# arpitbansal297/Cold-Diffusion-Models

Measured on AMD Instinct MI355X. Metric: unet_train_imgs_per_sec, higher is better.
Workload: dtype f32 storage/accumulate; dense-conv GEMM operands bf16x3; 1 GPU; CelebA-128 denoising cold diffusion (BASELINE config 3): Unet(dim=64,(1,2,4,8),ch=3) @128x128, T=200, optimizer step = 2 micro-batches x 32 img (one fused forward / backward pass over all of them: same draws, same gradient sum) + Adam + EMA/10; per_gpu_batch=32, gradient_accumulate_every=2, parallelism=single

## Files before the change

### cold-diffusion-models_amd/csrc/cdf_common.h

```cpp
#pragma once
#include <stdint.h>
#include <stddef.h>

#ifdef CDF_EMU
#include "hipemu.h"
#else
#include <hip/hip_runtime.h>
#define CDF_LAUNCH(kernel, grid, block, shmem, stream, ...) \
    hipLaunchKernelGGL(kernel, grid, block, shmem, stream, __VA_ARGS__)
#define CDF_DYN_SMEM(name) extern __shared__ __attribute__((aligned(16))) unsigned char name[]
#define CDF_LDS_BARRIER() asm volatile("s_waitcnt lgkmcnt(0)\n\ts_barrier" ::: "memory")
#define CDF_GLDS16(gptr, lds_base)                                                                            \
    __builtin_amdgcn_global_load_lds((const __attribute__((address_space(1))) void*)(gptr),                    \
                                     (__attribute__((address_space(3))) void*)(lds_base), 16, 0, 0)
#define CDF_WAIT_DMA() asm volatile("s_waitcnt vmcnt(0)" ::: "memory")
#define CDF_WAIT_DMA_LEAVE(N) asm volatile("s_waitcnt vmcnt(%0)" ::"n"(N) : "memory")
#define CDF_SCHED_FENCE() __builtin_amdgcn_sched_barrier(0)
#define CDF_WAIT_LDS() __builtin_amdgcn_s_waitcnt(0xC07F)
typedef float f32x4_t __attribute__((ext_vector_type(4)));
typedef float f32x16_t __attribute__((ext_vector_type(16)));
#endif
#ifdef CDF_EMU
#define CDF_LAUNCH_LDS_MAX(max_bytes, kernel, grid, block, shmem, stream, ...) CDF_LAUNCH(kernel, grid, block, shmem, stream, __VA_ARGS__)
#else
// ... 191 lines not shown
#define CDF_IO_RES_BF16 1
#define CDF_IO_PRE_BF16 2
#define CDF_IO_MUL_BF16 4
#define CDF_IO_PRE_GRAD 8

#define CDF_OK 0
#define CDF_E_INVALID (-1)
#define CDF_E_UNSUPPORTED (-2)
#define CDF_E_LAUNCH (-3)

#define CDF_WAVE 64
#define CDF_S ((hipStream_t)stream)

void cdf_set_error(const char* fmt, ...);
int cdf_check_launch(const char* what);

#define CDF_REQUIRE(cond, ...)                  \
    do {                                        \
        if (!(cond)) {                          \
            cdf_set_error(__VA_ARGS__);         \
            return CDF_E_INVALID;               \
        }                                       \
    } while (0)

static inline int cdf_cdiv(long long a, long long b) { return (int)((a + b - 1) / b); }

__device__ __forceinline__ int cdf_xcd_order(int bid, int nblk) {
    const int q = nblk >> 3, r = nblk & 7;
    const int xcd = bid & 7, idx = bid >> 3;
    const int base = xcd < r ? xcd * (q + 1) : r * (q + 1) + (xcd - r) * q;
// ... 65 lines not shown
```

### cold-diffusion-models_amd/csrc/k_conv.hip

```cpp
#include <atomic>
#include "cdf_common.h"
#include "cdf_epilogue.h"
#include "colddiff.h"

#define CDF_MAX_TAPS 16

struct ConvPhase {
    int oy, ox, ntaps;
    signed char dy[CDF_MAX_TAPS], dx[CDF_MAX_TAPS], wi[CDF_MAX_TAPS];
};

struct ConvArgs {
    const float* x;
    const float* w;
    float* y;
    const float* bias;
    const float* sbias;
    const float* res;
    float* pre;
    const float* mul;
    int ldx, ldw, ldy, ld_sbias, ldr, ldp, ldm;
    int B, H, W, Cin, OH, OW, Cout, QH, QW, os, is;
    int act;
    int mul_mode;
// ... 365 lines not shown
                           : a.out + (((long long)split * a.nbatch + batch) * a.ntaps + tap) * a.CA * a.ldo;
#pragma unroll
    for (int i = 0; i < MT; ++i)
#pragma unroll
        for (int r = 0; r < 16; ++r) {
            const int ca = tile_a * BMC + wm * WM + i * 32 + cdf_acc_row(r, half);
            if (ca >= a.CA) continue;
#pragma unroll
            for (int j = 0; j < NT; ++j) {
                const int cb = tile_b * BNC + wn * WN + j * 32 + l31;
                if (cb < a.ldo) O[(long long)ca * a.ldo + cb] = cb < a.CB ? acc[i][j][r] : 0.f;
            }
        }
}

__global__ void pack_weight_kernel(const float* src, float* dst, int T, int R, int C, int ldc, long long s_t,
                                   long long s_r, long long s_c) {
    const long long n = (long long)T * R * ldc;
    for (long long i = (long long)blockIdx.x * blockDim.x + threadIdx.x; i < n; i += (long long)gridDim.x * blockDim.x) {
        const int c = (int)(i % ldc);
        const long long tr = i / ldc;
        const int r = (int)(tr % R), t = (int)(tr / R);
        dst[i] = c < C ? src[c * s_c + r * s_r + t * s_t] : 0.f;
    }
}
template <int SL>
__global__ void __launch_bounds__(64 * SL) unpack_reduce_kernel(const float* ws, float* g, int nsplit, int T, int R, int C, int ldc,
                                                                long long s_t, long long s_r, long long s_c, int accumulate,
                                                                const float* bws, float* gb, int bC, int bld) {
    __shared__ float red[SL][64];
    if (bws != nullptr && blockIdx.y == 1) {
        ws = bws; g = gb; T = 1; R = 1; C = bC; ldc = bld; s_t = 0; s_r = 0; s_c = 1;
    }
    const long long n = (long long)T * R * C;
    const long long slab = (long long)T * R * ldc;
    const int l = threadIdx.x & 63, rl = threadIdx.x >> 6;
    for (long long base = (long long)blockIdx.x * 64; base < n; base += (long long)gridDim.x * 64) {
        const long long i = base + l;
        float s0 = 0.f, s1 = 0.f, s2 = 0.f, s3 = 0.f;
        int c = 0, r = 0, t = 0;
// ... 43 lines not shown
        tr = tile / tiles_c;
        tc = tile - tr * tiles_c;
    }
    const int c0 = tc * 32, r0 = tr * RJ;
    const long long slab = (long long)T_ * R * ldc;
    const int cc = c0 + cl < C ? c0 + cl : C - 1;
    int roff[J];
#pragma unroll
    for (int j = 0; j < J; ++j) {
        const int r = r0 + j / T_, t = j % T_;
        roff[j] = (t * R + (r < R ? r : R - 1)) * ldc + cc;
    }
    float acc[J];
#pragma unroll
    for (int j = 0; j < J; ++j) acc[j] = 0.f;
    for (int z = zg; z < nsplit; z += 8) {
        const float* p = ws + (long long)z * slab;
        float v[J];
#pragma unroll
        for (int j = 0; j < J; ++j) v[j] = p[roff[j]];
#pragma unroll
        for (int j = 0; j < J; ++j) acc[j] += v[j];
    }
#pragma unroll
    for (int j = 0; j < J; ++j) red[(zg * J + j) * 33 + cl] = acc[j];
    __syncthreads();
    constexpr int NE = (32 * J + 255) / 256;
    float tot[NE], old[NE];
    float* dst[NE];
    bool ok[NE];
#pragma unroll
// ... 55 lines not shown
        for (; r < r1; r += 4) s += cdf_widen(p[(long long)r * ld + c]);
    }
    red[rl][threadIdx.x & 63] = s;
    __syncthreads();
    if (rl == 0 && c < C) {
        const int l = threadIdx.x;
        part[((long long)blockIdx.y * gridDim.z + blockIdx.z) * C + c] = (red[0][l] + red[1][l]) + (red[2][l] + red[3][l]);
    }
}
__global__ void __launch_bounds__(1024) colsum_final_kernel(const float* part, float* out, int nchunk, int C, int ldo, int accumulate) {
    __shared__ float red[16][64];
    const int l = threadIdx.x & 63, rl = threadIdx.x >> 6, c = blockIdx.x * 64 + l;
    float s = 0.f;
    if (c < C) {
        const float* p = part + (long long)blockIdx.y * nchunk * C + c;
        for (int k = rl; k < nchunk; k += 16) s += p[(long long)k * C];
    }
    red[rl][l] = s;
    __syncthreads();
    if (rl == 0 && c < C) {
        float t = 0.f;
#pragma unroll
        for (int r = 0; r < 16; ++r) t += red[r][l];
        float* dst = out + (long long)blockIdx.y * ldo + c;
        *dst = accumulate ? *dst + t : t;
    }
}

static int check_feat(const char* who, const void* p, int ld, int C) {
    CDF_REQUIRE(p != nullptr, "%s: null tensor", who);
    CDF_REQUIRE((((uintptr_t)p) & 15) == 0, "%s: tensor not 16-byte aligned", who);
// ... 142 lines not shown

static inline int ew_grid2(long long n) {
    long long g = (n + 255) / 256;
    if (g > 4096) g = 4096;
    return g < 1 ? 1 : (int)g;
}

struct CdfPackEntry {
    const float* src;
    void* dst0;
    void* dst1;
    long long s_t, s_r, s_c;
    int T, R, C, ldc, kind, first_block;
};

__global__ void __launch_bounds__(256) pack_many_kernel(const CdfPackEntry* tab, int nentries) {
    int lo = 0, hi = nentries - 1;
    const int b = blockIdx.x;
    while (lo < hi) {
        const int mid = (lo + hi + 1) >> 1;
        if (tab[mid].first_block <= b) lo = mid; else hi = mid - 1;
    }
    const CdfPackEntry e = tab[lo];
    if (e.s_t == 1 && e.T > 1 && e.T <= 16) {
        const long long n2 = (long long)e.R * e.ldc;
        const long long j0 = (long long)(b - e.first_block) * 1024 + threadIdx.x;
        const long long plane = (long long)e.R * e.ldc;
#pragma unroll
        for (int k = 0; k < 4; ++k) {
            const long long j = j0 + 256 * k;
            if (j >= n2) break;
            const int c = (int)(j % e.ldc), r = (int)(j / e.ldc);
            const bool ok = c < e.C;
            const float* sp = e.src + (ok ? c * e.s_c + r * e.s_r : 0);
            float v[16];
#pragma unroll
            for (int t = 0; t < 16; ++t) v[t] = sp[t < e.T ? t : 0];
#pragma unroll
            for (int t = 0; t < 16; ++t) {
                if (t >= e.T) break;
                const float x = ok ? v[t] : 0.f;
                const long long i = t * plane + j;
                if (e.kind == 0) {
                    ((float*)e.dst0)[i] = x;
                } else {
                    const unsigned h = cdf_f2bf(x);
                    ((unsigned short*)e.dst0)[i] = (unsigned short)h;
                    if (e.dst1) ((unsigned short*)e.dst1)[i] = (unsigned short)cdf_f2bf(x - cdf_bf2f(h));
                }
            }
        }
        return;
    }
    const long long n = (long long)e.T * e.R * e.ldc;
    const long long i0 = (long long)(b - e.first_block) * 1024 + threadIdx.x;
#pragma unroll
    for (int k = 0; k < 4; ++k) {
        const long long i = i0 + 256 * k;
        if (i >= n) break;
        const int c = (int)(i % e.ldc);
        const long long tr = i / e.ldc;
        const int r = (int)(tr % e.R), t = (int)(tr / e.R);
        const float v = c < e.C ? e.src[c * e.s_c + r * e.s_r + t * e.s_t] : 0.f;
        if (e.kind == 0) {
            ((float*)e.dst0)[i] = v;
        } else {
            const unsigned h = cdf_f2bf(v);
            ((unsigned short*)e.dst0)[i] = (unsigned short)h;
            if (e.dst1) ((unsigned short*)e.dst1)[i] = (unsigned short)cdf_f2bf(v - cdf_bf2f(h));
        }
    }
}

extern "C" int cdf_pack_entry_bytes(void) { return (int)sizeof(CdfPackEntry); }
extern "C" int cdf_pack_blocks(int T, int R, int ldc, long long s_t) {
    const long long n = (s_t == 1 && T > 1 && T <= 16) ? (long long)R * ldc : (long long)T * R * ldc;
    return (int)((n + 1023) / 1024);
}

extern "C" int cdf_pack_many(const void* table, int nentries, int nblocks, void* stream) {
    CDF_REQUIRE(table && nentries > 0 && nblocks > 0, "cdf_pack_many: bad args");
    CDF_LAUNCH(pack_many_kernel, dim3(nblocks), dim3(256), 0, CDF_S, (const CdfPackEntry*)table, nentries);
    return cdf_check_launch("pack_many");
}

extern "C" int cdf_pack_weight(const float* src, float* dst, int T, int R, int C, int ldc, long long s_t,
                               long long s_r, long long s_c, void* stream) {
    CDF_REQUIRE(src && dst && T > 0 && R > 0 && C > 0 && ldc >= C && ldc % 4 == 0, "cdf_pack_weight: bad args");
    CDF_LAUNCH(pack_weight_kernel, dim3(ew_grid2((long long)T * R * ldc)), dim3(256), 0, CDF_S, src, dst, T, R, C, ldc, s_t, s_r, s_c);
    return cdf_check_launch("pack_weight");
}

static int launch_unpack_reduce(const float* ws, float* g, int nsplit, int T, int R, int C, int ldc, long long s_t, long long s_r,
                                long long s_c, int accumulate, const float* bws, float* gb, int bC, int bld, int tiled, hipStream_t s) {
    const int tiled_mode = tiled ? 1 : 0;
    if (s_c != 1 && C >= 32 && (T == 1 || T == 9 || T == 16) && tiled_mode) {
        const int RJ = T == 9 ? 4 : (T == 16 ? 2 : 32);
        const long long tiles = (long long)((C + 31) / 32) * ((R + RJ - 1) / RJ);
        if (tiles < (1 << 30) && (!bws || (bC + 31) / 32 <= tiles)) {
            const dim3 tg((unsigned)tiles, bws ? 2 : 1);
            if (T == 9)
                CDF_LAUNCH((unpack_reduce_tiled_kernel<9, 4>), tg, dim3(256), 0, s, ws, g, nsplit, R, C, ldc, s_t, s_r, s_c, accumulate, bws, gb, bC, bld, tiled_mode);
            else if (T == 16)
                CDF_LAUNCH((unpack_reduce_tiled_kernel<16, 2>), tg, dim3(256), 0, s, ws, g, nsplit, R, C, ldc, s_t, s_r, s_c, accumulate, bws, gb, bC, bld, tiled_mode);
            else
                CDF_LAUNCH((unpack_reduce_tiled_kernel<1, 32>), tg, dim3(256), 0, s, ws, g, nsplit, R, C, ldc, s_t, s_r, s_c, accumulate, bws, gb, bC, bld, tiled_mode);
            return cdf_check_launch("unpack_reduce_tiled");
        }
    }
    const dim3 grid(ew_grid2((long long)T * R * C * 4), bws ? 2 : 1);
    if (nsplit >= 32)
        CDF_LAUNCH(unpack_reduce_kernel<16>, grid, dim3(1024), 0, s, ws, g, nsplit, T, R, C, ldc, s_t, s_r, s_c, accumulate, bws, gb, bC, bld);
    else
        CDF_LAUNCH(unpack_reduce_kernel<4>, grid, dim3(256), 0, s, ws, g, nsplit, T, R, C, ldc, s_t, s_r, s_c, accumulate, bws, gb, bC, bld);
    return cdf_check_launch("unpack_reduce");
}

extern "C" int cdf_unpack_reduce(const float* ws, float* g, int nsplit, int T, int R, int C, int ldc, long long s_t,
                                 long long s_r, long long s_c, int accumulate, int tiled, void* stream) {
// ... 35 lines not shown
```

### cold-diffusion-models_amd/csrc/k_conv_sp.hip

```cpp
#include "cdf_conv_sp.h"
#include <atomic>

template <int SPLIT>
__global__ void __launch_bounds__(256, 2) conv_igemm_sp_kernel(SpArgs a) {
    constexpr int BM = 128, BN = 128, BK = 32, AS = 40;
    constexpr int NPL = SPLIT == 1 ? 1 : 2;
    constexpr int PLANE = BM * AS;
    constexpr int STAGE = 2 * NPL * PLANE;
    CDF_DYN_SMEM(smem_raw);
    unsigned short* smem = (unsigned short*)smem_raw;

    const int tid = threadIdx.x, lane = tid & 63, wave = tid >> 6;
    const int wm = wave >> 1, wn = wave & 1;
    const int M = a.B * a.QH * a.QW;
    const int tiles_n = (a.Cout + BN - 1) / BN, tiles_m = (M + BM - 1) / BM;
    const int tile = cdf_sp_swizzle(blockIdx.x, tiles_m * tiles_n);
    const int tile_m = tile / tiles_n, tile_n = tile - tile_m * tiles_n;
    const SpPhase& ph = a.ph[blockIdx.y];

    const int a_c4 = (tid & 7) * 4;
    int a_iy0[4], a_ix0[4];
    unsigned a_pix[4];
#pragma unroll
    for (int p = 0; p < 4; ++p) {
// ... 473 lines not shown
            }
        }
        __syncthreads();
    }
    psum += __shfl_xor(psum, 32);
    float* fold = stg;
    if (ctx_wave) {
        cdf_acc_stage(fold, LD, ch * LD, 0, cacc, half, l31);
        if (half == 0) fold[4 * LD * LD + ch * LD + l31] = psum;
    }
    __syncthreads();
    const size_t pb = (size_t)b * a.P + p;
    for (int e = tid; e < 4 * LD * LD; e += 512) a.ctx_part[pb * 4 * (LD * LD) + e] = t_lo < t_hi ? fold[e] : 0.f;
    if (tid < HD) a.sum_part[pb * HD + tid] = t_lo < t_hi ? fold[4 * LD * LD + tid] : 0.f;
    if (ctx_wave && half == 0) a.max_part[pb * HD + ch * LD + l31] = m_run;
}

__global__ void pack_weight_bf16_kernel(const float* src, unsigned short* dst_hi, unsigned short* dst_lo, int T, int R, int C,
                                        int ldc, long long s_t, long long s_r, long long s_c) {
    const long long n = (long long)T * R * ldc;
    for (long long i = (long long)blockIdx.x * blockDim.x + threadIdx.x; i < n; i += (long long)gridDim.x * blockDim.x) {
        const int c = (int)(i % ldc);
        const long long tr = i / ldc;
        const int r = (int)(tr % R), t = (int)(tr / R);
        const float v = c < C ? src[c * s_c + r * s_r + t * s_t] : 0.f;
        const unsigned h = cdf_f2bf(v);
        dst_hi[i] = (unsigned short)h;
        if (dst_lo) dst_lo[i] = (unsigned short)cdf_f2bf(v - cdf_bf2f(h));
    }
}

extern "C" int cdf_linattn_kvctx_parts(int B, int n, int slots) {
    const int tiles = n / 128;
    if (tiles < 1 || B < 1) return 0;
    int P = (slots > 0 ? slots : 512) / B;
    if (P < 1) P = 1;
    if (P > tiles) P = tiles;
    const int tpb = (tiles + P - 1) / P;
    return (tiles + tpb - 1) / tpb;
}

extern "C" int cdf_linattn_kvctx(const float* xn, int ldx, const void* w_hi, const void* w_lo, int ldk, float* kv, int ldkv, float* ws, int B,
                                 int n, int dim, int heads, int slots, void* stream) {
    CDF_REQUIRE(xn && w_hi && kv && ws && B > 0, "cdf_linattn_kvctx: null pointer");
// ... 12 lines not shown
    a.tiles_per_block = (tiles + P - 1) / P;
    const size_t lds = (size_t)128 * (256 + 8) * sizeof(float) + 8 * 32 * sizeof(float);
    if (dim % 64 == 0) {
        if (w_lo) CDF_LAUNCH_LDS((linattn_kvctx_kernel<3, 64>), dim3(P, B), dim3(512), lds, CDF_S, a);
        else CDF_LAUNCH_LDS((linattn_kvctx_kernel<1, 64>), dim3(P, B), dim3(512), lds, CDF_S, a);
    } else {
        if (w_lo) CDF_LAUNCH_LDS((linattn_kvctx_kernel<3, 32>), dim3(P, B), dim3(512), lds, CDF_S, a);
        else CDF_LAUNCH_LDS((linattn_kvctx_kernel<1, 32>), dim3(P, B), dim3(512), lds, CDF_S, a);
    }
    return cdf_check_launch("linattn_kvctx");
}

extern "C" int cdf_pack_weight_bf16(const float* src, void* dst_hi, void* dst_lo, int T, int R, int C, int ldc, long long s_t,
                                    long long s_r, long long s_c, void* stream) {
    CDF_REQUIRE(src && dst_hi && T > 0 && R > 0 && C > 0 && ldc >= C && ldc % 32 == 0, "cdf_pack_weight_bf16: bad args (ldc must be a multiple of 32)");
    long long g = ((long long)T * R * ldc + 255) / 256;
    if (g > 4096) g = 4096;
    CDF_LAUNCH(pack_weight_bf16_kernel, dim3((int)g), dim3(256), 0, CDF_S, src, (unsigned short*)dst_hi, (unsigned short*)dst_lo, T, R, C, ldc, s_t, s_r, s_c);
    return cdf_check_launch("pack_weight_bf16");
}

extern "C" int cdf_conv_gemm_bf16(const float* x, int ldx, const void* w_hi, const void* w_lo, int ldk, float* y, int ldy, int B,
                                  int H, int W, int Cin, int OH, int OW, int Cout, int QH, int QW, int os, int is, int nphase,
                                  const int* phase_desc, const float* bias, const float* sbias, int ld_sbias, const float* res,
                                  int ldr, float* pre, int ldp, const float* mul, int ldm, int act, int mul_mode, int accumulate,
                                  int split, void* stream) {
    CDF_REQUIRE(x && w_hi && y && (((uintptr_t)x) & 15) == 0 && ldx % 4 == 0 && ldx >= Cin, "cdf_conv_gemm_bf16: bad x");
    CDF_REQUIRE((split == 1 || split == 3) && (split == 1 || w_lo), "cdf_conv_gemm_bf16: split must be 1 (bf16) or 3 (hi/lo bf16x3)");
    CDF_REQUIRE((((uintptr_t)w_hi) & 15) == 0 && ldk % 32 == 0 && ldk >= Cin, "cdf_conv_gemm_bf16: weights must be 16B aligned with ldk %% 32 == 0");
    CDF_REQUIRE(nphase >= 1 && nphase <= 4 && phase_desc && ldy >= Cout, "cdf_conv_gemm_bf16: bad geometry");
    CDF_REQUIRE(!mul_mode || mul, "cdf_conv_gemm_bf16: mul_mode without mul tensor");
    SpArgs a;
    a.x = x; a.w_hi = (const unsigned short*)w_hi; a.w_lo = (const unsigned short*)w_lo; a.y = y;
    a.bias = bias; a.sbias = sbias; a.res = res; a.pre = pre; a.mul = mul;
// ... 72 lines not shown
```

### cold-diffusion-models_amd/csrc/k_dwconv.hip

```cpp
#include <type_traits>
#include "cdf_common.h"
#include "colddiff.h"

#define DW_K 7
#define DW_TAPS 49

__device__ __forceinline__ void f4_fma(float4& acc, const float4& a, const float4& b) {
    acc.x = fmaf(a.x, b.x, acc.x);
    acc.y = fmaf(a.y, b.y, acc.y);
    acc.z = fmaf(a.z, b.z, acc.z);
    acc.w = fmaf(a.w, b.w, acc.w);
}

template <int TBW, int TBH, bool BF, bool YB = BF>
__global__ void __launch_bounds__(256, 2) dwconv7_kernel(const void* x, int ldx, const float* w, int ldw, const float* bias,
                                                         const float* sbias, int ld_sbias, void* y, int ldy, int B, int H,
                                                         int W, int C4, int flip, int accumulate, const void* res, int ldr,
                                                         void* y_hi, void* y_lo, int ld_ys) {
    typedef typename cdf_quad<BF>::raw raw_t;
    typedef typename cdf_quad<BF>::elem elem_t;
    typedef typename cdf_quad<YB>::elem yelem_t;
    constexpr int HW_ = TBW + 6, HH_ = TBH + 6;
    constexpr int RP = HW_ * 8 + 4;
    constexpr int TX = TBW / 4, TY = TBH / 2;
// ... 388 lines not shown
            if (c + 2 < C) p[2] = v.z;
            if (c + 3 < C) p[3] = v.w;
        }
    };
#pragma unroll
    for (int r = 0; r < 2; ++r)
#pragma unroll
        for (int kx = 0; kx < DW_K; ++kx) {
            fold(acc[r][kx]);
            if (r < nky) put((ky0 + r) * DW_K + kx, acc[r][kx]);
        }
    fold(dsum);
    if (wave == 3) put(DW_TAPS, dsum);
}

__global__ void __launch_bounds__(1024) dwconv7_wgrad_final_kernel(const float* part, int B, int nchunk, int C, float* dw, float* dbias,
                                                                  float* dsb, int ld_dsb, int accumulate) {
    __shared__ float red[16][64];
    const int l = threadIdx.x & 63, rl = threadIdx.x >> 6, c = blockIdx.x * 64 + l, t = blockIdx.y;
    const int n = B * nchunk;
    float s0 = 0.f, s1 = 0.f;
    if (c < C) {
        int i = rl;
        for (; i + 16 < n; i += 32) {
            s0 += part[((long long)i * (DW_TAPS + 1) + t) * C + c];
            s1 += part[((long long)(i + 16) * (DW_TAPS + 1) + t) * C + c];
        }
        if (i < n) s0 += part[((long long)i * (DW_TAPS + 1) + t) * C + c];
    }
    red[rl][l] = s0 + s1;
    __syncthreads();
    if (rl == 0 && c < C) {
        float tot = 0.f;
#pragma unroll
        for (int r = 0; r < 16; ++r) tot += red[r][l];
        if (t < DW_TAPS) {
            float* dst = dw + (long long)c * DW_TAPS + t;
            *dst = accumulate ? *dst + tot : tot;
        } else if (dbias) {
            dbias[c] = accumulate ? dbias[c] + tot : tot;
        }
    }
    if (t == DW_TAPS && dsb) {
        __syncthreads();
        for (int b = rl; b < B; b += 16) {
            if (c < C) {
                float sb = 0.f;
                for (int k = 0; k < nchunk; ++k) sb += part[(((long long)b * nchunk + k) * (DW_TAPS + 1) + DW_TAPS) * C + c];
                dsb[(long long)b * ld_dsb + c] = sb;
            }
        }
    }
}

template <int TBW, int TBH, bool BF, bool YB = BF>
static int launch_dwconv7(const void* x, int ldx, const float* w, int ldw, const float* bias, const float* sbias, int ld_sbias, void* y,
                          int ldy, int B, int H, int W, int C4, int flip, int accumulate, const void* res, int ldr, hipStream_t s,
                          void* y_hi = nullptr, void* y_lo = nullptr, int ld_ys = 0) {
    constexpr size_t lds = ((size_t)(TBH + 6) * ((TBW + 6) * 8 + 4) + DW_TAPS * 8) * sizeof(float4);
    const long long tiles = (long long)B * cdf_cdiv(H, TBH) * cdf_cdiv(W, TBW);
    CDF_LAUNCH_LDS((dwconv7_kernel<TBW, TBH, BF, YB>), dim3((unsigned)tiles, cdf_cdiv(C4, 8)), dim3(256), lds, s, x, ldx, w, ldw, bias, sbias, ld_sbias, y,
               ldy, B, H, W, C4, flip, accumulate, res, ldr, y_hi, y_lo, ld_ys);
    return cdf_check_launch("dwconv7");
}
// ... 59 lines not shown
    CDF_REQUIRE(ldx % 4 == 0 && lddy % 4 == 0 && ldx >= ((C + 3) & ~3) && lddy >= ((C + 3) & ~3) && ((((uintptr_t)x) | ((uintptr_t)dy)) & (io_bf16 ? 7 : 15)) == 0,
                "cdf_dwconv7_wgrad: pitches must be multiples of 4 and >= roundup4(C), pointers 16B aligned (bf16: 8B)");
    {
        const long long ldmax = ldx > lddy ? ldx : lddy;
        CDF_REQUIRE(W < 32 || ((long long)H * W < (1 << 24) && ldmax < (1 << 24) && (long long)H * W * ldmax < (1LL << 30)),
                    "cdf_dwconv7_wgrad: image of %d x %d pixels at pitch %lld is beyond the kernel's 32-bit per-image offsets", H, W, ldmax);
    }
    const int nchunk = cdf_dwconv7_wgrad_nchunk(H), rpc = cdf_cdiv(H, nchunk);
    if (W >= 32) {
        if (io_bf16) CDF_LAUNCH(dwconv7_wgrad_partial_kernel<true>, dim3(cdf_cdiv(C, 32), nchunk, B), dim3(256), 0, CDF_S, x, ldx, dy, lddy, ws, H, W, C, rpc);
        else CDF_LAUNCH(dwconv7_wgrad_partial_kernel<false>, dim3(cdf_cdiv(C, 32), nchunk, B), dim3(256), 0, CDF_S, x, ldx, dy, lddy, ws, H, W, C, rpc);
    } else {
        if (io_bf16) CDF_LAUNCH(dwconv7_wgrad_partial_narrow_kernel<true>, dim3(cdf_cdiv(C, 64), nchunk, B), dim3(256), 0, CDF_S, x, ldx, dy, lddy, ws, H, W, C, rpc);
        else CDF_LAUNCH(dwconv7_wgrad_partial_narrow_kernel<false>, dim3(cdf_cdiv(C, 64), nchunk, B), dim3(256), 0, CDF_S, x, ldx, dy, lddy, ws, H, W, C, rpc);
    }
    CDF_LAUNCH(dwconv7_wgrad_final_kernel, dim3(cdf_cdiv(C, 64), DW_TAPS + 1), dim3(1024), 0, CDF_S, (const float*)ws, B, nchunk, C, dw, dbias, dsb, ld_dsb, accumulate);
    return cdf_check_launch("dwconv7_wgrad");
}

extern "C" int cdf_dwconv7_wgrad(const float* x, int ldx, const float* dy, int lddy, float* dw, float* dbias,
                                 float* dsb, int ld_dsb, float* ws, int B, int H, int W, int C, int accumulate,
                                 void* stream) {
    return cdf_dwconv7_wgrad_io(x, ldx, dy, lddy, dw, dbias, dsb, ld_dsb, ws, B, H, W, C, accumulate, 0, stream);
}
```

### cold-diffusion-models_amd/csrc/k_norm.hip

```cpp
#include "cdf_common.h"
#include "colddiff.h"

template <int NV, bool XB>
__global__ void __launch_bounds__(256) layernorm_c_fwd_kernel(const void* x, int ldx, float* y, int ldy, const float* g,
                                                              const float* bta, float* mean_out, float* rstd_out,
                                                              long long M, int C, int LP, float eps, unsigned short* ys_hi,
                                                              unsigned short* ys_lo, int ld_ys) {
    constexpr int U = NV <= 2 ? 4 : 2;
    const int lane = threadIdx.x & 63, sub = lane / LP, li = lane - sub * LP;
    const int groups_per_wave = 64 / LP;
    const long long wave_global = ((long long)blockIdx.x * blockDim.x + threadIdx.x) >> 6;
    const long long nwaves = ((long long)gridDim.x * blockDim.x) >> 6;
    const long long npg = (M + groups_per_wave - 1) / groups_per_wave;
    float4 gg[NV], bb[NV];
#pragma unroll
    for (int j = 0; j < NV; ++j) {
        const int c = (li + j * LP) * 4;
        gg[j] = *(const float4*)(g + (c < C ? c : 0));
        bb[j] = *(const float4*)(bta + (c < C ? c : 0));
    }
    for (long long pg0 = wave_global * U; pg0 < npg; pg0 += nwaves * U) {
        float4 v[U][NV];
#pragma unroll
        for (int u = 0; u < U; ++u) {
// ... 151 lines not shown
    for (int j = 0; j < NV; ++j) {
        const int c = (li + j * LP) * 4;
        if (c < C) {
            *(float4*)(sred + ((size_t)gidx * 2 + 0) * C + c) = adg[j];
            *(float4*)(sred + ((size_t)gidx * 2 + 1) * C + c) = adb[j];
        }
    }
    __syncthreads();
    for (int i = threadIdx.x; i < 2 * C; i += blockDim.x) {
        float s = 0.f;
        for (int gg2 = 0; gg2 < G; ++gg2) s += sred[(size_t)gg2 * 2 * C + i];
        part[(size_t)blockIdx.x * 2 * C + i] = s;
    }
}

__global__ void __launch_bounds__(1024) norm_param_reduce_kernel(const float* part, int nblocks, int C, float* dg, float* db, int accumulate) {
    __shared__ float red[16][64];
    const int l = threadIdx.x & 63, rl = threadIdx.x >> 6, i = blockIdx.x * 64 + l;
    float s0 = 0.f, s1 = 0.f;
    if (i < 2 * C) {
        float t0 = 0.f, t1 = 0.f, t2 = 0.f, t3 = 0.f, t4 = 0.f, t5 = 0.f, t6 = 0.f, t7 = 0.f;
        const float* p = part + i;
        const size_t st = (size_t)2 * C;
        int b = rl;
        for (; b + 112 < nblocks; b += 128) {
            const float v0 = p[(size_t)b * st], v1 = p[(size_t)(b + 16) * st], v2 = p[(size_t)(b + 32) * st], v3 = p[(size_t)(b + 48) * st];
            const float v4 = p[(size_t)(b + 64) * st], v5 = p[(size_t)(b + 80) * st], v6 = p[(size_t)(b + 96) * st], v7 = p[(size_t)(b + 112) * st];
            t0 += v0; t1 += v1; t2 += v2; t3 += v3; t4 += v4; t5 += v5; t6 += v6; t7 += v7;
        }
        for (; b + 16 < nblocks; b += 32) {
            s0 += p[(size_t)b * st];
            s1 += p[(size_t)(b + 16) * st];
        }
        if (b < nblocks) s0 += p[(size_t)b * st];
        s0 += (t0 + t1) + (t2 + t3);
        s1 += (t4 + t5) + (t6 + t7);
    }
    red[rl][l] = s0 + s1;
    __syncthreads();
    if (rl == 0 && i < 2 * C) {
        float t = 0.f;
#pragma unroll
        for (int r = 0; r < 16; ++r) t += red[r][l];
        float* dst = i < C ? dg + i : db + (i - C);
        *dst = accumulate ? *dst + t : t;
    }
}

__global__ void groupnorm_partial_kernel(const float* x, int ldx, const float* dy, int lddy, const float* gamma,
                                         const float* beta, const float* mean, const float* rstd, float* part, int HW,
                                         int rows_per_chunk, int C, int groups, int mode, int silu, float p_drop,
                                         unsigned long long seed) {
    const unsigned thr = (unsigned)((double)p_drop * 4294967296.0);
    const float inv = 1.0f / (1.0f - p_drop);
    __shared__ float red[2][4][64];
    const int c = blockIdx.x * 64 + (threadIdx.x & 63), rl = threadIdx.x >> 6, b = blockIdx.z;
    const int r0 = blockIdx.y * rows_per_chunk;
    int r1 = r0 + rows_per_chunk;
    if (r1 > HW) r1 = HW;
    float p0 = 0.f, p1 = 0.f;
// ... 254 lines not shown
    CDF_REQUIRE(ln_geometry(C, &LP, &NV) == CDF_OK, "cdf_layernorm_c_bwd: unsupported C=%d", C);
    const int nb = cdf_layernorm_blocks(M, C);
    const int G = 4 * (64 / LP);
    const size_t lds = (size_t)G * 2 * C * sizeof(float);
#define CDF_LN_BWD(N, IO) CDF_LAUNCH_LDS((layernorm_c_bwd_kernel<N, IO>), dim3(nb), dim3(256), lds, CDF_S, dy, lddy, x, ldx, g, mean, rstd, dx, lddx, part, M, C, LP, add, ldadd, (unsigned short*)dx_hi, (unsigned short*)dx_lo, ld_planes)
#define CDF_LN_BWD_NV(IO)                  \
    switch (NV) {                          \
        case 1: CDF_LN_BWD(1, IO); break;  \
        case 2: CDF_LN_BWD(2, IO); break;  \
        case 3: CDF_LN_BWD(3, IO); break;  \
        default: CDF_LN_BWD(4, IO); break; \
    }
    if (io_bf16 == 7) { CDF_LN_BWD_NV(7) } else if (io_bf16 == 14) { CDF_LN_BWD_NV(14) } else { CDF_LN_BWD_NV(0) }
#undef CDF_LN_BWD_NV
#undef CDF_LN_BWD
    CDF_LAUNCH(norm_param_reduce_kernel, dim3(cdf_cdiv(2 * C, 64)), dim3(1024), 0, CDF_S, (const float*)part, nb, C, dg, db, accumulate_param);
    return cdf_check_launch("layernorm_c_bwd");
}

extern "C" int cdf_norm_param_reduce(const float* part, int nblocks, int C, float* dg, float* db, int accumulate, void* stream) {
    CDF_REQUIRE(part && dg && db && nblocks > 0 && C > 0, "cdf_norm_param_reduce: bad args");
    CDF_LAUNCH(norm_param_reduce_kernel, dim3(cdf_cdiv(2 * C, 64)), dim3(1024), 0, CDF_S, part, nblocks, C, dg, db, accumulate);
    return cdf_check_launch("norm_param_reduce");
}

extern "C" int cdf_layernorm_c_bwd_io(const void* dy, int lddy, const void* x, int ldx, const float* g,
                                      const float* mean, const float* rstd, void* dx, int lddx, const void* add, int ldadd,
                                      float* dg, float* db, float* part, long long M, int C, int accumulate_dx, int accumulate_param,
                                      int io_bf16, void* stream) {
    return ln_bwd_launch(dy, lddy, x, ldx, g, mean, rstd, dx, lddx, add, ldadd, dg, db, part, M, C, accumulate_dx, accumulate_param, io_bf16, nullptr, nullptr, 0, stream);
}
extern "C" int cdf_layernorm_c_bwd_planes(const float* dy, int lddy, const float* x, int ldx, const float* g, const float* mean, const float* rstd,
                                          float* dx, int lddx, const float* add, int ldadd, float* dg, float* db, float* part, long long M, int C,
                                          int accumulate_dx, int accumulate_param, void* dx_hi, void* dx_lo, int ld_planes, void* stream) {
    return ln_bwd_launch(dy, lddy, x, ldx, g, mean, rstd, dx, lddx, add, ldadd, dg, db, part, M, C, accumulate_dx, accumulate_param, 0, dx_hi, dx_lo, ld_planes, stream);
}

// ... 71 lines not shown
```

Measured before the change: 1275 img/s.

## Restructure weight packing and gradient reduction kernels for memory-level parallelism

Replaces the per-format weight pack kernels with one shared pack path. That path uses an LDS-tiled transpose for strided weights and paired vector stores, and can run as a single-entry launch. Several split-K and partial-sum reduction kernels (unpack_reduce_tiled, colsum_final, dwconv7 wgrad final, norm_param_reduce) are unrolled to keep more independent loads in flight, and some are re-gridded so more blocks cover fewer columns. These steps are small memory-bound kernels that sit around each conv weight update. The changes add code complexity and LDS use in the pack kernel.

```diff
diff --git a/cold-diffusion-models_amd/csrc/cdf_common.h b/cold-diffusion-models_amd/csrc/cdf_common.h
--- a/cold-diffusion-models_amd/csrc/cdf_common.h
+++ b/cold-diffusion-models_amd/csrc/cdf_common.h
@@ -229,6 +229,8 @@
 
 void cdf_set_error(const char* fmt, ...);
 int cdf_check_launch(const char* what);
+int cdf_pack_launch_one(const float* src, void* dst0, void* dst1, int T, int R, int C, int ldc, long long s_t, long long s_r, long long s_c,
+                        int kind, void* stream, const char* who);
 
 #define CDF_REQUIRE(cond, ...)                  \
     do {                                        \
diff --git a/cold-diffusion-models_amd/csrc/k_conv.hip b/cold-diffusion-models_amd/csrc/k_conv.hip
--- a/cold-diffusion-models_amd/csrc/k_conv.hip
+++ b/cold-diffusion-models_amd/csrc/k_conv.hip
@@ -403,16 +403,6 @@
         }
 }
 
-__global__ void pack_weight_kernel(const float* src, float* dst, int T, int R, int C, int ldc, long long s_t,
-                                   long long s_r, long long s_c) {
-    const long long n = (long long)T * R * ldc;
-    for (long long i = (long long)blockIdx.x * blockDim.x + threadIdx.x; i < n; i += (long long)gridDim.x * blockDim.x) {
-        const int c = (int)(i % ldc);
-        const long long tr = i / ldc;
-        const int r = (int)(tr % R), t = (int)(tr / R);
-        dst[i] = c < C ? src[c * s_c + r * s_r + t * s_t] : 0.f;
-    }
-}
 template <int SL>
 __global__ void __launch_bounds__(64 * SL) unpack_reduce_kernel(const float* ws, float* g, int nsplit, int T, int R, int C, int ldc,
                                                                 long long s_t, long long s_r, long long s_c, int accumulate,
@@ -486,7 +476,20 @@
     float acc[J];
 #pragma unroll
     for (int j = 0; j < J; ++j) acc[j] = 0.f;
-    for (int z = zg; z < nsplit; z += 8) {
+    constexpr int U = J >= 16 ? 1 : 16 / J;
+    int z = zg;
+    for (; z + 8 * (U - 1) < nsplit; z += 8 * U) {
+        float v[U][J];
+#pragma unroll
+        for (int u = 0; u < U; ++u)
+#pragma unroll
+            for (int j = 0; j < J; ++j) v[u][j] = ws[(long long)(z + 8 * u) * slab + roff[j]];
+#pragma unroll
+        for (int u = 0; u < U; ++u)
+#pragma unroll
+            for (int j = 0; j < J; ++j) acc[j] += v[u][j];
+    }
+    for (; z < nsplit; z += 8) {
         const float* p = ws + (long long)z * slab;
         float v[J];
 #pragma unroll
@@ -572,7 +575,14 @@
     float s = 0.f;
     if (c < C) {
         const float* p = part + (long long)blockIdx.y * nchunk * C + c;
-        for (int k = rl; k < nchunk; k += 16) s += p[(long long)k * C];
+        for (int k = rl; k < nchunk; k += 16 * 8) {
+            float v[8];
+#pragma unroll
+            for (int u = 0; u < 8; ++u) v[u] = p[(long long)(k + 16 * u < nchunk ? k + 16 * u : k) * C];
+#pragma unroll
+            for (int u = 0; u < 8; ++u)
+                if (k + 16 * u < nchunk) s += v[u];
+        }
     }
     red[rl][l] = s;
     __syncthreads();
@@ -745,17 +755,115 @@
     int T, R, C, ldc, kind, first_block;
 };
 
-__global__ void __launch_bounds__(256) pack_many_kernel(const CdfPackEntry* tab, int nentries) {
-    int lo = 0, hi = nentries - 1;
-    const int b = blockIdx.x;
-    while (lo < hi) {
-        const int mid = (lo + hi + 1) >> 1;
-        if (tab[mid].first_block <= b) lo = mid; else hi = mid - 1;
-    }
-    const CdfPackEntry e = tab[lo];
-    if (e.s_t == 1 && e.T > 1 && e.T <= 16) {
+#define PACK_TC 64
+#define PACK_TL 144
+#define PACK_LDS (PACK_TC * (PACK_TL | 1))
+
+__host__ __device__ static inline bool pack_taps_whole(int T, long long s_t) { return s_t == 1 && T > 1 && T <= 16; }
+__host__ __device__ static inline long long pack_nblocks(int T, int R, int ldc, long long s_t) {
+    const long long n = pack_taps_whole(T, s_t) ? (long long)R * ldc : (long long)T * R * ldc;
+    return (n + 1023) / 1024;
+}
+
+__device__ __forceinline__ void pack_put(const CdfPackEntry& e, long long i, float x) {
+    if (e.kind == 0) {
+        ((float*)e.dst0)[i] = x;
+    } else {
+        const unsigned h = cdf_f2bf(x);
+        ((unsigned short*)e.dst0)[i] = (unsigned short)h;
+        if (e.dst1) ((unsigned short*)e.dst1)[i] = (unsigned short)cdf_f2bf(x - cdf_bf2f(h));
+    }
+}
+
+__device__ __forceinline__ void pack_put2(const CdfPackEntry& e, long long i, float x0, float x1) {
+    if (e.kind == 0) {
+        *(float2*)((float*)e.dst0 + i) = make_float2(x0, x1);
+    } else {
+        const unsigned h0 = cdf_f2bf(x0), h1 = cdf_f2bf(x1);
+        *(unsigned*)((unsigned short*)e.dst0 + i) = h0 | (h1 << 16);
+        if (e.dst1) *(unsigned*)((unsigned short*)e.dst1 + i) = cdf_f2bf(x0 - cdf_bf2f(h0)) | (cdf_f2bf(x1 - cdf_bf2f(h1)) << 16);
+    }
+}
+__device__ __forceinline__ bool pack_pairs_ok(const CdfPackEntry& e) {
+    const uintptr_t m = e.kind == 0 ? 7 : 3;
+    return (e.ldc & 1) == 0 && ((((uintptr_t)e.dst0) | ((uintptr_t)e.dst1)) & m) == 0;
+}
+
+__device__ __forceinline__ void pack_entry_body(const CdfPackEntry& e, int blk, int nblk, float* tile) {
+    const bool whole = pack_taps_whole(e.T, e.s_t);
+    const bool pairs = pack_pairs_ok(e);
+    if ((whole || e.T == 1) && e.R > 1 && e.s_r < e.s_c && pairs) {
+        const int T = e.T;
+        int RT = 64;
+        while (RT * T > PACK_TL) RT >>= 1;
+        const int L = RT * T, P = L | 1;
+        const int tiles_c = (e.ldc + PACK_TC - 1) / PACK_TC, tiles_r = (e.R + RT - 1) / RT;
+        const int ntiles = tiles_c * tiles_r;
+        const int lane = threadIdx.x & 63, wave = threadIdx.x >> 6;
+        int q[3];
+        long long qoff[3];
+#pragma unroll
+        for (int k = 0; k < 3; ++k) {
+            q[k] = lane + 64 * k;
+            const int r = q[k] / T, t = q[k] - r * T;
+            qoff[k] = r * e.s_r + t * e.s_t;
+        }
+        for (int tile_i = blk; tile_i < ntiles; tile_i += nblk) {
+            const int vt = cdf_xcd_order(tile_i, ntiles);
+            const int tc = vt / tiles_r, tr = vt - tc * tiles_r;
+            const int c0 = tc * PACK_TC, r0 = tr * RT;
+            const int qlim = (e.R - r0) * T < L ? (e.R - r0) * T : L;
+            for (int i0 = 0; i0 < PACK_TC / 4; i0 += 4)
+#pragma unroll
+            for (int i = i0; i < i0 + 4; ++i) {
+                const int cl = wave + 4 * i;
+                const bool okc = c0 + cl < e.C;
+                const float* sp = e.src + (okc ? (c0 + cl) * e.s_c : 0) + r0 * e.s_r;
+#pragma unroll
+                for (int k = 0; k < 3; ++k) {
+                    const bool ok = okc && q[k] < qlim;
+                    const float v = sp[ok ? qoff[k] : 0];
+                    if (q[k] < L) tile[cl * P + q[k]] = ok ? v : 0.f;
+                }
+            }
+            __syncthreads();
+            const int cp = 2 * (lane & 31), rh = lane >> 5;
+            const int rend = e.R - r0 < RT ? e.R - r0 : RT;
+            if (c0 + cp < e.ldc) {
+                for (int t = 0; t < T; ++t)
+                    for (int r = 2 * wave + rh; r < rend; r += 8)
+                        pack_put2(e, ((long long)t * e.R + r0 + r) * e.ldc + c0 + cp, tile[cp * P + r * T + t], tile[(cp + 1) * P + r * T + t]);
+            }
+            __syncthreads();
+        }
+        return;
+    }
+    if (whole && pairs) {
         const long long n2 = (long long)e.R * e.ldc;
-        const long long j0 = (long long)(b - e.first_block) * 1024 + threadIdx.x;
+        const long long j0 = (long long)blk * 1024 + 2 * threadIdx.x;
+#pragma unroll
+        for (int k = 0; k < 2; ++k) {
+            const long long j = j0 + 512 * k;
+            if (j >= n2) break;
+            const int c = (int)(j % e.ldc), r = (int)(j / e.ldc);
+            const bool ok0 = c < e.C, ok1 = c + 1 < e.C;
+            const float* sp0 = e.src + (ok0 ? c * e.s_c + r * e.s_r : 0);
+            const float* sp1 = e.src + (ok1 ? (c + 1) * e.s_c + r * e.s_r : 0);
+            float v0[16], v1[16];
+#pragma unroll
+            for (int t = 0; t < 16; ++t) {
+                v0[t] = sp0[t < e.T ? t : 0];
+                v1[t] = sp1[t < e.T ? t : 0];
+            }
+#pragma unroll
+            for (int t = 0; t < 16; ++t)
+                if (t < e.T) pack_put2(e, t * n2 + j, ok0 ? v0[t] : 0.f, ok1 ? v1[t] : 0.f);
+        }
+        return;
+    }
+    if (whole) {
+        const long long n2 = (long long)e.R * e.ldc;
+        const long long j0 = (long long)blk * 1024 + threadIdx.x;
         const long long plane = (long long)e.R * e.ldc;
 #pragma unroll
         for (int k = 0; k < 4; ++k) {
@@ -768,23 +876,13 @@
 #pragma unroll
             for (int t = 0; t < 16; ++t) v[t] = sp[t < e.T ? t : 0];
 #pragma unroll
-            for (int t = 0; t < 16; ++t) {
-                if (t >= e.T) break;
-                const float x = ok ? v[t] : 0.f;
-                const long long i = t * plane + j;
-                if (e.kind == 0) {
-                    ((float*)e.dst0)[i] = x;
-                } else {
-                    const unsigned h = cdf_f2bf(x);
-                    ((unsigned short*)e.dst0)[i] = (unsigned short)h;
-                    if (e.dst1) ((unsigned short*)e.dst1)[i] = (unsigned short)cdf_f2bf(x - cdf_bf2f(h));
-                }
-            }
+            for (int t = 0; t < 16; ++t)
+                if (t < e.T) pack_put(e, t * plane + j, ok ? v[t] : 0.f);
         }
         return;
     }
     const long long n = (long long)e.T * e.R * e.ldc;
-    const long long i0 = (long long)(b - e.first_block) * 1024 + threadIdx.x;
+    const long long i0 = (long long)blk * 1024 + threadIdx.x;
 #pragma unroll
     for (int k = 0; k < 4; ++k) {
         const long long i = i0 + 256 * k;
@@ -792,22 +890,28 @@
         const int c = (int)(i % e.ldc);
         const long long tr = i / e.ldc;
         const int r = (int)(tr % e.R), t = (int)(tr / e.R);
-        const float v = c < e.C ? e.src[c * e.s_c + r * e.s_r + t * e.s_t] : 0.f;
-        if (e.kind == 0) {
-            ((float*)e.dst0)[i] = v;
-        } else {
-            const unsigned h = cdf_f2bf(v);
-            ((unsigned short*)e.dst0)[i] = (unsigned short)h;
-            if (e.dst1) ((unsigned short*)e.dst1)[i] = (unsigned short)cdf_f2bf(v - cdf_bf2f(h));
-        }
-    }
+        pack_put(e, i, c < e.C ? e.src[c * e.s_c + r * e.s_r + t * e.s_t] : 0.f);
+    }
+}
+
+__global__ void __launch_bounds__(256) pack_many_kernel(const CdfPackEntry* tab, int nentries) {
+    __shared__ float tile[PACK_LDS];
+    int lo = 0, hi = nentries - 1;
+    const int b = blockIdx.x;
+    while (lo < hi) {
+        const int mid = (lo + hi + 1) >> 1;
+        if (tab[mid].first_block <= b) lo = mid; else hi = mid - 1;
+    }
+    const CdfPackEntry e = tab[lo];
+    pack_entry_body(e, b - e.first_block, (int)pack_nblocks(e.T, e.R, e.ldc, e.s_t), tile);
+}
+__global__ void __launch_bounds__(256) pack_one_kernel(CdfPackEntry e) {
+    __shared__ float tile[PACK_LDS];
+    pack_entry_body(e, blockIdx.x, gridDim.x, tile);
 }
 
 extern "C" int cdf_pack_entry_bytes(void) { return (int)sizeof(CdfPackEntry); }
-extern "C" int cdf_pack_blocks(int T, int R, int ldc, long long s_t) {
-    const long long n = (s_t == 1 && T > 1 && T <= 16) ? (long long)R * ldc : (long long)T * R * ldc;
-    return (int)((n + 1023) / 1024);
-}
+extern "C" int cdf_pack_blocks(int T, int R, int ldc, long long s_t) { return (int)pack_nblocks(T, R, ldc, s_t); }
 
 extern "C" int cdf_pack_many(const void* table, int nentries, int nblocks, void* stream) {
     CDF_REQUIRE(table && nentries > 0 && nblocks > 0, "cdf_pack_many: bad args");
@@ -815,18 +919,29 @@
     return cdf_check_launch("pack_many");
 }
 
+int cdf_pack_launch_one(const float* src, void* dst0, void* dst1, int T, int R, int C, int ldc, long long s_t, long long s_r, long long s_c,
+                        int kind, void* stream, const char* who) {
+    const long long nblk = pack_nblocks(T, R, ldc, s_t);
+    CDF_REQUIRE(nblk < (1LL << 31), "%s: layout too large", who);
+    CdfPackEntry e;
+    e.src = src; e.dst0 = dst0; e.dst1 = dst1; e.s_t = s_t; e.s_r = s_r; e.s_c = s_c;
+    e.T = T; e.R = R; e.C = C; e.ldc = ldc; e.kind = kind; e.first_block = 0;
+    CDF_LAUNCH(pack_one_kernel, dim3((unsigned)nblk), dim3(256), 0, CDF_S, e);
+    return cdf_check_launch(who);
+}
+
 extern "C" int cdf_pack_weight(const float* src, float* dst, int T, int R, int C, int ldc, long long s_t,
                                long long s_r, long long s_c, void* stream) {
     CDF_REQUIRE(src && dst && T > 0 && R > 0 && C > 0 && ldc >= C && ldc % 4 == 0, "cdf_pack_weight: bad args");
-    CDF_LAUNCH(pack_weight_kernel, dim3(ew_grid2((long long)T * R * ldc)), dim3(256), 0, CDF_S, src, dst, T, R, C, ldc, s_t, s_r, s_c);
-    return cdf_check_launch("pack_weight");
+    return cdf_pack_launch_one(src, dst, nullptr, T, R, C, ldc, s_t, s_r, s_c, 0, stream, "pack_weight");
 }
 
 static int launch_unpack_reduce(const float* ws, float* g, int nsplit, int T, int R, int C, int ldc, long long s_t, long long s_r,
                                 long long s_c, int accumulate, const float* bws, float* gb, int bC, int bld, int tiled, hipStream_t s) {
     const int tiled_mode = tiled ? 1 : 0;
     if (s_c != 1 && C >= 32 && (T == 1 || T == 9 || T == 16) && tiled_mode) {
-        const int RJ = T == 9 ? 4 : (T == 16 ? 2 : 32);
+        const long long tiles_c1 = (C + 31) / 32;
+        const int RJ = T == 9 ? 4 : (T == 16 ? 2 : (tiles_c1 * ((R + 31) / 32) >= 1024 ? 32 : (tiles_c1 * ((R + 3) / 4) >= 512 ? 4 : 1)));
         const long long tiles = (long long)((C + 31) / 32) * ((R + RJ - 1) / RJ);
         if (tiles < (1 << 30) && (!bws || (bC + 31) / 32 <= tiles)) {
             const dim3 tg((unsigned)tiles, bws ? 2 : 1);
@@ -834,6 +949,10 @@
                 CDF_LAUNCH((unpack_reduce_tiled_kernel<9, 4>), tg, dim3(256), 0, s, ws, g, nsplit, R, C, ldc, s_t, s_r, s_c, accumulate, bws, gb, bC, bld, tiled_mode);
             else if (T == 16)
                 CDF_LAUNCH((unpack_reduce_tiled_kernel<16, 2>), tg, dim3(256), 0, s, ws, g, nsplit, R, C, ldc, s_t, s_r, s_c, accumulate, bws, gb, bC, bld, tiled_mode);
+            else if (RJ == 4)
+                CDF_LAUNCH((unpack_reduce_tiled_kernel<1, 4>), tg, dim3(256), 0, s, ws, g, nsplit, R, C, ldc, s_t, s_r, s_c, accumulate, bws, gb, bC, bld, tiled_mode);
+            else if (RJ == 1)
+                CDF_LAUNCH((unpack_reduce_tiled_kernel<1, 1>), tg, dim3(256), 0, s, ws, g, nsplit, R, C, ldc, s_t, s_r, s_c, accumulate, bws, gb, bC, bld, tiled_mode);
             else
                 CDF_LAUNCH((unpack_reduce_tiled_kernel<1, 32>), tg, dim3(256), 0, s, ws, g, nsplit, R, C, ldc, s_t, s_r, s_c, accumulate, bws, gb, bC, bld, tiled_mode);
             return cdf_check_launch("unpack_reduce_tiled");
diff --git a/cold-diffusion-models_amd/csrc/k_conv_sp.hip b/cold-diffusion-models_amd/csrc/k_conv_sp.hip
--- a/cold-diffusion-models_amd/csrc/k_conv_sp.hip
+++ b/cold-diffusion-models_amd/csrc/k_conv_sp.hip
@@ -511,20 +511,6 @@
     for (int e = tid; e < 4 * LD * LD; e += 512) a.ctx_part[pb * 4 * (LD * LD) + e] = t_lo < t_hi ? fold[e] : 0.f;
     if (tid < HD) a.sum_part[pb * HD + tid] = t_lo < t_hi ? fold[4 * LD * LD + tid] : 0.f;
     if (ctx_wave && half == 0) a.max_part[pb * HD + ch * LD + l31] = m_run;
-}
-
-__global__ void pack_weight_bf16_kernel(const float* src, unsigned short* dst_hi, unsigned short* dst_lo, int T, int R, int C,
-                                        int ldc, long long s_t, long long s_r, long long s_c) {
-    const long long n = (long long)T * R * ldc;
-    for (long long i = (long long)blockIdx.x * blockDim.x + threadIdx.x; i < n; i += (long long)gridDim.x * blockDim.x) {
-        const int c = (int)(i % ldc);
-        const long long tr = i / ldc;
-        const int r = (int)(tr % R), t = (int)(tr / R);
-        const float v = c < C ? src[c * s_c + r * s_r + t * s_t] : 0.f;
-        const unsigned h = cdf_f2bf(v);
-        dst_hi[i] = (unsigned short)h;
-        if (dst_lo) dst_lo[i] = (unsigned short)cdf_f2bf(v - cdf_bf2f(h));
-    }
 }
 
 extern "C" int cdf_linattn_kvctx_parts(int B, int n, int slots) {
@@ -567,10 +553,7 @@
 extern "C" int cdf_pack_weight_bf16(const float* src, void* dst_hi, void* dst_lo, int T, int R, int C, int ldc, long long s_t,
                                     long long s_r, long long s_c, void* stream) {
     CDF_REQUIRE(src && dst_hi && T > 0 && R > 0 && C > 0 && ldc >= C && ldc % 32 == 0, "cdf_pack_weight_bf16: bad args (ldc must be a multiple of 32)");
-    long long g = ((long long)T * R * ldc + 255) / 256;
-    if (g > 4096) g = 4096;
-    CDF_LAUNCH(pack_weight_bf16_kernel, dim3((int)g), dim3(256), 0, CDF_S, src, (unsigned short*)dst_hi, (unsigned short*)dst_lo, T, R, C, ldc, s_t, s_r, s_c);
-    return cdf_check_launch("pack_weight_bf16");
+    return cdf_pack_launch_one(src, dst_hi, dst_lo, T, R, C, ldc, s_t, s_r, s_c, 1, stream, "pack_weight_bf16");
 }
 
 extern "C" int cdf_conv_gemm_bf16(const float* x, int ldx, const void* w_hi, const void* w_lo, int ldk, float* y, int ldy, int B,
diff --git a/cold-diffusion-models_amd/csrc/k_dwconv.hip b/cold-diffusion-models_amd/csrc/k_dwconv.hip
--- a/cold-diffusion-models_amd/csrc/k_dwconv.hip
+++ b/cold-diffusion-models_amd/csrc/k_dwconv.hip
@@ -426,40 +426,97 @@
     if (wave == 3) put(DW_TAPS, dsum);
 }
 
-__global__ void __launch_bounds__(1024) dwconv7_wgrad_final_kernel(const float* part, int B, int nchunk, int C, float* dw, float* dbias,
-                                                                  float* dsb, int ld_dsb, int accumulate) {
-    __shared__ float red[16][64];
-    const int l = threadIdx.x & 63, rl = threadIdx.x >> 6, c = blockIdx.x * 64 + l, t = blockIdx.y;
+#define DW_FU 16
+#define DW_FP 64
+template <int V> struct dw_vec { typedef float type; };
+template <> struct dw_vec<4> { typedef float4 type; };
+__device__ __forceinline__ void dw_vec_get(float* o, const float& v) { o[0] = v; }
+__device__ __forceinline__ void dw_vec_get(float* o, const float4& v) { o[0] = v.x; o[1] = v.y; o[2] = v.z; o[3] = v.w; }
+template <int V>
+__global__ void __launch_bounds__(256) dwconv7_wgrad_final_kernel(const float* part, int B, int nchunk, int C, float* dw, float* dbias,
+                                                                 float* dsb, int ld_dsb, int accumulate) {
+    typedef typename dw_vec<V>::type vec_t;
+    __shared__ float red[DW_FP / 16][4 * V];
+    const int cl = threadIdx.x & 3, pl = threadIdx.x >> 2, wave = threadIdx.x >> 6;
+    const int c = (blockIdx.x * 4 + cl) * V, t = blockIdx.y;
     const int n = B * nchunk;
-    float s0 = 0.f, s1 = 0.f;
-    if (c < C) {
-        int i = rl;
-        for (; i + 16 < n; i += 32) {
-            s0 += part[((long long)i * (DW_TAPS + 1) + t) * C + c];
-            s1 += part[((long long)(i + 16) * (DW_TAPS + 1) + t) * C + c];
-        }
-        if (i < n) s0 += part[((long long)i * (DW_TAPS + 1) + t) * C + c];
-    }
-    red[rl][l] = s0 + s1;
+    const bool okc = c < C;
+    const long long st = (long long)(DW_TAPS + 1) * C;
+    if (t > DW_TAPS) {
+        if (!dsb) return;
+        for (int b = pl; b < B; b += DW_FP) {
+            const float* q = part + ((long long)b * nchunk * (DW_TAPS + 1) + DW_TAPS) * C + (okc ? c : 0);
+            float sb[V];
+#pragma unroll
+            for (int v = 0; v < V; ++v) sb[v] = 0.f;
+            for (int k0 = 0; k0 < nchunk; k0 += 32) {
+                vec_t x[32];
+#pragma unroll
+                for (int u = 0; u < 32; ++u) x[u] = *(const vec_t*)(q + (k0 + u < nchunk ? k0 + u : k0) * st);
+#pragma unroll
+                for (int u = 0; u < 32; ++u) {
+                    float f[V];
+                    dw_vec_get(f, x[u]);
+                    if (k0 + u < nchunk)
+#pragma unroll
+                        for (int v = 0; v < V; ++v) sb[v] += f[v];
+                }
+            }
+            if (okc)
+#pragma unroll
+                for (int v = 0; v < V; ++v) dsb[(long long)b * ld_dsb + c + v] = sb[v];
+        }
+        return;
+    }
+    const float* p = part + (long long)t * C + (okc ? c : 0);
+    float acc[DW_FU][V];
+#pragma unroll
+    for (int u = 0; u < DW_FU; ++u)
+#pragma unroll
+        for (int v = 0; v < V; ++v) acc[u][v] = 0.f;
+    for (int i0 = pl; i0 < n; i0 += DW_FP * DW_FU) {
+        vec_t x[DW_FU];
+#pragma unroll
+        for (int u = 0; u < DW_FU; ++u) {
+            const int i = i0 + DW_FP * u;
+            x[u] = *(const vec_t*)(p + (i < n ? i : i0) * st);
+        }
+#pragma unroll
+        for (int u = 0; u < DW_FU; ++u) {
+            float f[V];
+            dw_vec_get(f, x[u]);
+            const bool ok = okc && i0 + DW_FP * u < n;
+#pragma unroll
+            for (int v = 0; v < V; ++v) acc[u][v] += ok ? f[v] : 0.f;
+        }
+    }
+    float s[V];
+#pragma unroll
+    for (int v = 0; v < V; ++v) {
+#pragma unroll
+        for (int w = 1; w < DW_FU; w <<= 1)
+#pragma unroll
+            for (int u = 0; u < DW_FU; u += 2 * w) acc[u][v] += acc[u + w][v];
+        s[v] = acc[0][v];
+#pragma unroll
+        for (int o = 4; o < 64; o <<= 1) s[v] += __shfl_xor(s[v], o);
+    }
+    if ((threadIdx.x & 63) < 4)
+#pragma unroll
+        for (int v = 0; v < V; ++v) red[wave][cl * V + v] = s[v];
     __syncthreads();
-    if (rl == 0 && c < C) {
+    if (threadIdx.x < 4 * V) {
+        const int ch = blockIdx.x * 4 * V + threadIdx.x;
         float tot = 0.f;
 #pragma unroll
-        for (int r = 0; r < 16; ++r) tot += red[r][l];
-        if (t < DW_TAPS) {
-            float* dst = dw + (long long)c * DW_TAPS + t;
-            *dst = accumulate ? *dst + tot : tot;
-        } else if (dbias) {
-            dbias[c] = accumulate ? dbias[c] + tot : tot;
-        }
-    }
-    if (t == DW_TAPS && dsb) {
-        __syncthreads();
-        for (int b = rl; b < B; b += 16) {
-            if (c < C) {
-                float sb = 0.f;
-                for (int k = 0; k < nchunk; ++k) sb += part[(((long long)b * nchunk + k) * (DW_TAPS + 1) + DW_TAPS) * C + c];
-                dsb[(long long)b * ld_dsb + c] = sb;
+        for (int w = 0; w < DW_FP / 16; w += 4)
+            tot += (red[w][threadIdx.x] + red[w + 1][threadIdx.x]) + (red[w + 2][threadIdx.x] + red[w + 3][threadIdx.x]);
+        if (ch < C) {
+            if (t < DW_TAPS) {
+                float* dst = dw + (long long)ch * DW_TAPS + t;
+                *dst = accumulate ? *dst + tot : tot;
+            } else if (dbias) {
+                dbias[ch] = accumulate ? dbias[ch] + tot : tot;
             }
         }
     }
@@ -549,7 +606,10 @@
         if (io_bf16) CDF_LAUNCH(dwconv7_wgrad_partial_narrow_kernel<true>, dim3(cdf_cdiv(C, 64), nchunk, B), dim3(256), 0, CDF_S, x, ldx, dy, lddy, ws, H, W, C, rpc);
         else CDF_LAUNCH(dwconv7_wgrad_partial_narrow_kernel<false>, dim3(cdf_cdiv(C, 64), nchunk, B), dim3(256), 0, CDF_S, x, ldx, dy, lddy, ws, H, W, C, rpc);
     }
-    CDF_LAUNCH(dwconv7_wgrad_final_kernel, dim3(cdf_cdiv(C, 64), DW_TAPS + 1), dim3(1024), 0, CDF_S, (const float*)ws, B, nchunk, C, dw, dbias, dsb, ld_dsb, accumulate);
+    if (C % 4 == 0 && (((uintptr_t)ws) & 15) == 0)
+        CDF_LAUNCH(dwconv7_wgrad_final_kernel<4>, dim3(cdf_cdiv(C, 16), DW_TAPS + 2), dim3(256), 0, CDF_S, (const float*)ws, B, nchunk, C, dw, dbias, dsb, ld_dsb, accumulate);
+    else
+        CDF_LAUNCH(dwconv7_wgrad_final_kernel<1>, dim3(cdf_cdiv(C, 4), DW_TAPS + 2), dim3(256), 0, CDF_S, (const float*)ws, B, nchunk, C, dw, dbias, dsb, ld_dsb, accumulate);
     return cdf_check_launch("dwconv7_wgrad");
 }
 
diff --git a/cold-diffusion-models_amd/csrc/k_norm.hip b/cold-diffusion-models_amd/csrc/k_norm.hip
--- a/cold-diffusion-models_amd/csrc/k_norm.hip
+++ b/cold-diffusion-models_amd/csrc/k_norm.hip
@@ -189,36 +189,45 @@
     }
 }
 
+#define NP_U 16
 __global__ void __launch_bounds__(1024) norm_param_reduce_kernel(const float* part, int nblocks, int C, float* dg, float* db, int accumulate) {
-    __shared__ float red[16][64];
-    const int l = threadIdx.x & 63, rl = threadIdx.x >> 6, i = blockIdx.x * 64 + l;
-    float s0 = 0.f, s1 = 0.f;
-    if (i < 2 * C) {
-        float t0 = 0.f, t1 = 0.f, t2 = 0.f, t3 = 0.f, t4 = 0.f, t5 = 0.f, t6 = 0.f, t7 = 0.f;
-        const float* p = part + i;
-        const size_t st = (size_t)2 * C;
-        int b = rl;
-        for (; b + 112 < nblocks; b += 128) {
-            const float v0 = p[(size_t)b * st], v1 = p[(size_t)(b + 16) * st], v2 = p[(size_t)(b + 32) * st], v3 = p[(size_t)(b + 48) * st];
-            const float v4 = p[(size_t)(b + 64) * st], v5 = p[(size_t)(b + 80) * st], v6 = p[(size_t)(b + 96) * st], v7 = p[(size_t)(b + 112) * st];
-            t0 += v0; t1 += v1; t2 += v2; t3 += v3; t4 += v4; t5 += v5; t6 += v6; t7 += v7;
-        }
-        for (; b + 16 < nblocks; b += 32) {
-            s0 += p[(size_t)b * st];
-            s1 += p[(size_t)(b + 16) * st];
-        }
-        if (b < nblocks) s0 += p[(size_t)b * st];
-        s0 += (t0 + t1) + (t2 + t3);
-        s1 += (t4 + t5) + (t6 + t7);
-    }
-    red[rl][l] = s0 + s1;
+    __shared__ float red[16][16];
+    const int cl = threadIdx.x & 15, pl = threadIdx.x >> 4, wave = threadIdx.x >> 6, i = blockIdx.x * 16 + cl;
+    const bool ok = i < 2 * C;
+    const float* p = part + (ok ? i : 0);
+    const size_t st = (size_t)2 * C;
+    float t[NP_U];
+#pragma unroll
+    for (int u = 0; u < NP_U; ++u) t[u] = 0.f;
+    for (int b0 = pl; b0 < nblocks; b0 += 64 * NP_U) {
+        float v[NP_U];
+#pragma unroll
+        for (int u = 0; u < NP_U; ++u) {
+            const int b = b0 + 64 * u;
+            v[u] = p[(size_t)(b < nblocks ? b : b0) * st];
+        }
+#pragma unroll
+        for (int u = 0; u < NP_U; ++u) t[u] += b0 + 64 * u < nblocks ? v[u] : 0.f;
+    }
+#pragma unroll
+    for (int w = 1; w < NP_U; w <<= 1)
+#pragma unroll
+        for (int u = 0; u < NP_U; u += 2 * w) t[u] += t[u + w];
+    float s = t[0];
+    s += __shfl_xor(s, 16);
+    s += __shfl_xor(s, 32);
+    if ((threadIdx.x & 63) < 16) red[wave][cl] = s;
     __syncthreads();
-    if (rl == 0 && i < 2 * C) {
-        float t = 0.f;
-#pragma unroll
-        for (int r = 0; r < 16; ++r) t += red[r][l];
+    if (threadIdx.x < 16 && ok) {
+        float r[16];
+#pragma unroll
+        for (int w = 0; w < 16; ++w) r[w] = red[w][cl];
+#pragma unroll
+        for (int w = 1; w < 16; w <<= 1)
+#pragma unroll
+            for (int u = 0; u < 16; u += 2 * w) r[u] += r[u + w];
         float* dst = i < C ? dg + i : db + (i - C);
-        *dst = accumulate ? *dst + t : t;
+        *dst = accumulate ? *dst + r[0] : r[0];
     }
 }
 
@@ -503,13 +512,13 @@
     if (io_bf16 == 7) { CDF_LN_BWD_NV(7) } else if (io_bf16 == 14) { CDF_LN_BWD_NV(14) } else { CDF_LN_BWD_NV(0) }
 #undef CDF_LN_BWD_NV
 #undef CDF_LN_BWD
-    CDF_LAUNCH(norm_param_reduce_kernel, dim3(cdf_cdiv(2 * C, 64)), dim3(1024), 0, CDF_S, (const float*)part, nb, C, dg, db, accumulate_param);
+    CDF_LAUNCH(norm_param_reduce_kernel, dim3(cdf_cdiv(2 * C, 16)), dim3(1024), 0, CDF_S, (const float*)part, nb, C, dg, db, accumulate_param);
     return cdf_check_launch("layernorm_c_bwd");
 }
 
 extern "C" int cdf_norm_param_reduce(const float* part, int nblocks, int C, float* dg, float* db, int accumulate, void* stream) {
     CDF_REQUIRE(part && dg && db && nblocks > 0 && C > 0, "cdf_norm_param_reduce: bad args");
-    CDF_LAUNCH(norm_param_reduce_kernel, dim3(cdf_cdiv(2 * C, 64)), dim3(1024), 0, CDF_S, part, nblocks, C, dg, db, accumulate);
+    CDF_LAUNCH(norm_param_reduce_kernel, dim3(cdf_cdiv(2 * C, 16)), dim3(1024), 0, CDF_S, part, nblocks, C, dg, db, accumulate);
     return cdf_check_launch("norm_param_reduce");
 }
 
```

Measured after the change: 1283 img/s (median of 6 runs). Within noise of the previous version (+0.6%).
